# AIM-SE/AC-TSR

Measured on AMD Instinct MI355X. Metric: user-sequences/sec fwd+bwd, AC-SASRec L=50 d=64, 1/2/4/8 MI355X, higher is better.
Workload: dtype f32; 1 GPU; ACSASRec full training step (spatial + adversarial calibrators, BASELINE configs[2]), synthetic 100000-item catalogue, B=512/GPU L=50 d=64 h=2 2 layers inner=256, CE loss, two-pass backward + Adam; global_batch=512, seq_len=50, hidden=64, heads=2, parallelism=dp1, launch=hipGraph replay per step, backward=two walks (reference protocol, trainer.py:672-686)

## Files before the change

ac_tsr_amd/csrc/acattn_linear.hip:

```cpp
#include <stdlib.h>

#include <algorithm>

#include "acattn_common.h"
#include "acattn_sumrows.h"

namespace {

constexpr int kRegs = 64;

struct WgradGroup {
  const float* x[ACATTN_WGRAD_MAX_GROUP];
  const float* dy[ACATTN_WGRAD_MAX_GROUP];
  float* dw[ACATTN_WGRAD_MAX_GROUP];
  float* db[ACATTN_WGRAD_MAX_GROUP];
  int K[ACATTN_WGRAD_MAX_GROUP];
  int N[ACATTN_WGRAD_MAX_GROUP];
  long long w_off[ACATTN_WGRAD_MAX_GROUP];
  long long b_off[ACATTN_WGRAD_MAX_GROUP];
};

__device__ __forceinline__ f4 load_rows4(const float* base, int64_t row, int64_t M, int ld, int col, int ncols) {
  f4 v = {0.f, 0.f, 0.f, 0.f};
  if (row < M) {
    const float* p = base + row * ld + col;
    if (col + 3 < ncols) {
      v = *(const f4u*)p;
    } else {
#pragma unroll
      for (int e = 0; e < 4; ++e)
        if (col + e < ncols) v[e] = p[e];
    }
  }
  return v;
}

template <int UNROLL>
__global__ void __launch_bounds__(256, 2) wgrad_partial_kernel(const WgradGroup G, const int64_t M,
                                                             float* __restrict__ ws) {
  const int it = blockIdx.z;
  const int K = G.K[it], N = G.N[it];
  const int KB = (K + 63) >> 6, NB = (N + 63) >> 6;
  if ((int)blockIdx.y >= KB * NB) return;
  const float* __restrict__ x = G.x[it];
  const float* __restrict__ dy = G.dy[it];
  float* part_w = ws + G.w_off[it];
  float* part_b = G.db[it] ? ws + G.b_off[it] : nullptr;
  const int lane = threadIdx.x & 63, wave = threadIdx.x >> 6;
  const int c = lane & 15, g = lane >> 4;
  const int blk = blockIdx.y, nb = blk / KB, kb = blk - nb * KB;
  const int P = gridDim.x;
  const int ncol = nb * 64 + 4 * c, kcol = kb * 64 + 4 * c;

  f4 acc[4][4];
#pragma unroll
  for (int a = 0; a < 4; ++a)
#pragma unroll
    for (int b = 0; b < 4; ++b) acc[a][b] = f4{0.f, 0.f, 0.f, 0.f};
  f4 bsum = {0.f, 0.f, 0.f, 0.f};

  const int64_t stride = (int64_t)P * 4 * 4, batch = stride * UNROLL;
  int64_t m0 = ((int64_t)blockIdx.x * 4 + wave) * 4;
  if ((K & 63) == 0 && (N & 63) == 0) {
    auto load_batch = [&](int64_t r0, f4 (&xv)[UNROLL], f4 (&gv)[UNROLL]) {
#pragma unroll
      for (int u = 0; u < UNROLL; ++u) {
        const int64_t row = min(r0 + u * stride + g, M - 1);
        xv[u] = *(const f4*)(x + row * K + kcol);
        gv[u] = *(const f4*)(dy + row * N + ncol);
      }
    };
    auto mma_batch = [&](int64_t r0, const f4 (&xv)[UNROLL], const f4 (&gv)[UNROLL]) {
#pragma unroll
      for (int u = 0; u < UNROLL; ++u) {
        const bool row_in = r0 + u * stride + g < M;
        f4 gq;
#pragma unroll
        for (int e = 0; e < 4; ++e) gq[e] = row_in ? gv[u][e] : 0.f;
        bsum += gq;
#pragma unroll
        for (int a = 0; a < 4; ++a)
#pragma unroll
          for (int b = 0; b < 4; ++b) acc[a][b] = mfma16(gq[a], xv[u][b], acc[a][b]);
      }
    };
    f4 xa[UNROLL], ga[UNROLL], xb[UNROLL], gb[UNROLL];
    load_batch(m0, xa, ga);
#pragma nounroll
    for (; m0 < M; m0 += 2 * batch) {
      load_batch(m0 + batch, xb, gb);
      __builtin_amdgcn_sched_barrier(0);
      mma_batch(m0, xa, ga);
      load_batch(m0 + 2 * batch, xa, ga);
      __builtin_amdgcn_sched_barrier(0);
      if (m0 + batch < M) mma_batch(m0 + batch, xb, gb);
    }
  } else {
    for (; m0 < M; m0 += batch) {
      f4 xv[UNROLL], gv[UNROLL];
#pragma unroll
      for (int u = 0; u < UNROLL; ++u) {
        const int64_t row = m0 + u * stride + g;
        xv[u] = load_rows4(x, row, M, K, kcol, K);
        gv[u] = load_rows4(dy, row, M, N, ncol, N);
      }
#pragma unroll
      for (int u = 0; u < UNROLL; ++u) {
        bsum += gv[u];
#pragma unroll
        for (int a = 0; a < 4; ++a)
#pragma unroll
          for (int b = 0; b < 4; ++b) acc[a][b] = mfma16(gv[u][a], xv[u][b], acc[a][b]);
      }
    }
  }

  __shared__ float red[4 * kRegs * 64];
#pragma unroll
  for (int a = 0; a < 4; ++a)
#pragma unroll
    for (int b = 0; b < 4; ++b)
#pragma unroll
      for (int r = 0; r < 4; ++r) red[(wave * kRegs + (a * 4 + b) * 4 + r) * 64 + lane] = acc[a][b][r];
  __syncthreads();
  float* pw = part_w + ((size_t)blk * P + blockIdx.x) * (kRegs * 64);
  for (int s = threadIdx.x; s < kRegs * 64; s += 256)
    pw[s] = (red[s] + red[kRegs * 64 + s]) + (red[2 * kRegs * 64 + s] + red[3 * kRegs * 64 + s]);
  if (part_b && kb == 0) {
    __syncthreads();
    *(f4*)(red + 4 * threadIdx.x) = bsum;
    __syncthreads();
    if (threadIdx.x < 64) {
      float s = 0.f;
#pragma unroll
      for (int wg = 0; wg < 16; ++wg) s += red[4 * (wg * 16 + (threadIdx.x >> 2)) + (threadIdx.x & 3)];
      part_b[((size_t)nb * P + blockIdx.x) * 64 + threadIdx.x] = s;
    }
  }
}

__global__ void __launch_bounds__(256) wgrad_reduce_kernel(const WgradGroup G, const float* __restrict__ ws,
                                                            const int P) {
  const int it = blockIdx.z;
  const int K = G.K[it], N = G.N[it];
  const int KB = (K + 63) >> 6, NB = (N + 63) >> 6;
  if ((int)blockIdx.y >= KB * NB) return;
  float* __restrict__ dw = G.dw[it];
  float* __restrict__ db = G.db[it];
  const float* part_w = ws + G.w_off[it];
  const float* part_b = ws + G.b_off[it];
  const int blk = blockIdx.y, nb = blk / KB, kb = blk - nb * KB;
  const int sl = threadIdx.x & 31, q = threadIdx.x >> 5;
  const int s = blockIdx.x * 32 + sl;
  const float* pw = part_w + (size_t)blk * P * (kRegs * 64) + s;
  constexpr size_t PS = kRegs * 64;
  float a[8];
#pragma unroll
  for (int u = 0; u < 8; ++u) a[u] = 0.f;
  int p = q;
  for (; p + 56 < P; p += 64) {
#pragma unroll
    for (int u = 0; u < 8; ++u) a[u] += pw[(size_t)(p + 8 * u) * PS];
  }
  for (; p < P; p += 8) a[0] += pw[(size_t)p * PS];
  __shared__ float red[8][32];
  red[q][sl] = ((a[0] + a[1]) + (a[2] + a[3])) + ((a[4] + a[5]) + (a[6] + a[7]));
  __syncthreads();
  if (q == 0) {
    float v = 0.f;
#pragma unroll
    for (int u = 0; u < 8; ++u) v += red[u][sl];
    const int reg = s >> 6, lane = s & 63;
    const int tile = reg >> 2, r = reg & 3, aa = tile >> 2, bb = tile & 3, g = lane >> 4, c = lane & 15;
    const int n = nb * 64 + 4 * (4 * g + r) + aa, k = kb * 64 + 4 * c + bb;
    if (n < N && k < K) dw[(size_t)n * K + k] = v;
  }
  if (db && kb == 0 && blockIdx.x < 2) {
    __syncthreads();
    const int col = blockIdx.x * 32 + sl, nn = nb * 64 + col;
    const float* pb = part_b + (size_t)nb * P * 64 + col;
    float sb = 0.f;
    for (int t = q; t < P; t += 8) sb += pb[(size_t)t * 64];
    red[q][sl] = sb;
    __syncthreads();
    if (q == 0 && nn < N) {
      float v = 0.f;
#pragma unroll
      for (int u = 0; u < 8; ++u) v += red[u][sl];
      db[nn] = v;
    }
  }
}

struct WgradMany {
  const float* part_w[ACATTN_WGRAD_MAX_REDUCE];
  const float* part_b[ACATTN_WGRAD_MAX_REDUCE];
  float* dw[ACATTN_WGRAD_MAX_REDUCE];
  float* db[ACATTN_WGRAD_MAX_REDUCE];
  int K[ACATTN_WGRAD_MAX_REDUCE];
  int N[ACATTN_WGRAD_MAX_REDUCE];
  int P[ACATTN_WGRAD_MAX_REDUCE];
  SumRowsJob sr[ACATTN_SUMROWS_MAX_DEFER];
  int n_w;
};

__global__ void __launch_bounds__(256) wgrad_reduce_many_kernel(const WgradMany G) {
  if ((int)blockIdx.z >= G.n_w) {
    const SumRowsJob& j = G.sr[blockIdx.z - G.n_w];
    const int w = blockIdx.y * gridDim.x + blockIdx.x;
    if (w < j.n_wg) sum_rows_block<false>(j.x, j.out, j.R, j.C, j.R, j.CT, w % j.col_groups, 0, w / j.col_groups);
    return;
  }
  const int it = blockIdx.z;
  const int K = G.K[it], N = G.N[it];
  const int KB = (K + 63) >> 6, NB = (N + 63) >> 6;
  if ((int)blockIdx.y >= KB * NB) return;
  float* __restrict__ dw = G.dw[it];
  float* __restrict__ db = G.db[it];
  const float* part_w = G.part_w[it];
  const float* part_b = G.part_b[it];
  const int P = G.P[it];
  const int blk = blockIdx.y, nb = blk / KB, kb = blk - nb * KB;
  const int sl = threadIdx.x & 31, q = threadIdx.x >> 5;
  const int s = blockIdx.x * 32 + sl;
  const float* pw = part_w + (size_t)blk * P * (kRegs * 64) + s;
  constexpr size_t PS = kRegs * 64;
  float a[8];
#pragma unroll
  for (int u = 0; u < 8; ++u) a[u] = 0.f;
  int p = q;
  for (; p + 56 < P; p += 64) {
#pragma unroll
    for (int u = 0; u < 8; ++u) a[u] += pw[(size_t)(p + 8 * u) * PS];
  }
  for (; p < P; p += 8) a[0] += pw[(size_t)p * PS];
  __shared__ float red[8][32];
  red[q][sl] = ((a[0] + a[1]) + (a[2] + a[3])) + ((a[4] + a[5]) + (a[6] + a[7]));
  __syncthreads();
  if (q == 0) {
    float v = 0.f;
#pragma unroll
    for (int u = 0; u < 8; ++u) v += red[u][sl];
    const int reg = s >> 6, lane = s & 63;
    const int tile = reg >> 2, r = reg & 3, aa = tile >> 2, bb = tile & 3, g = lane >> 4, c = lane & 15;
    const int n = nb * 64 + 4 * (4 * g + r) + aa, k = kb * 64 + 4 * c + bb;
    if (n < N && k < K) dw[(size_t)n * K + k] = v;
  }
  if (db && kb == 0 && blockIdx.x < 2) {
    __syncthreads();
    const int col = blockIdx.x * 32 + sl, nn = nb * 64 + col;
    const float* pb = part_b + (size_t)nb * P * 64 + col;
    float sb = 0.f;
    for (int t = q; t < P; t += 8) sb += pb[(size_t)t * 64];
    red[q][sl] = sb;
    __syncthreads();
    if (q == 0 && nn < N) {
      float v = 0.f;
#pragma unroll
      for (int u = 0; u < 8; ++u) v += red[u][sl];
      db[nn] = v;
    }
  }
}

int pick_partials(int64_t M, int blocks) {
  static const int forced = getenv("ACATTN_WGRAD_PARTIALS") ? atoi(getenv("ACATTN_WGRAD_PARTIALS")) : 0;
  int p = forced > 0 ? forced : std::max(64, 128 / blocks);
  return (int)std::min<int64_t>(p, std::max<int64_t>(1, M / 64));
}

}

namespace {
int64_t item_ws_floats(int K, int N, int P) {
  const int64_t KB = (K + 63) / 64, NB = (N + 63) / 64;
  return KB * NB * P * kRegs * 64 + NB * P * 64;
}
int group_partials(int64_t M, const int* K, const int* N, int n_items) {
  int blocks = 1;
  for (int i = 0; i < n_items; ++i) blocks = std::max(blocks, ((K[i] + 63) / 64) * ((N[i] + 63) / 64));
  return pick_partials(M, blocks);
}
}

int64_t acattn_linear_wgrad_ws_bytes(int64_t M, int K, int N) {
  return item_ws_floats(K, N, pick_partials(M, 1)) * (int64_t)sizeof(float);
}

int acattn_launch_linear_wgrad(const float* const* x, const float* const* dy, const int* K, const int* N,
                               float* const* dw, float* const* db, int n_items, int64_t M, void* ws, hipStream_t stream,
                               int* P_out, long long* w_off_out, long long* b_off_out) {
  WgradGroup G{};
  const int P = group_partials(M, K, N, n_items);
  int blocks = 1;
  long long off = 0;
  for (int i = 0; i < n_items; ++i) {
    G.x[i] = x[i];
    G.dy[i] = dy[i];
    G.dw[i] = dw[i];
    G.db[i] = db[i];
    G.K[i] = K[i];
    G.N[i] = N[i];
    const long long KB = (K[i] + 63) / 64, NB = (N[i] + 63) / 64;
    G.w_off[i] = off;
    G.b_off[i] = off + KB * NB * P * kRegs * 64;
    off += item_ws_floats(K[i], N[i], P);
    blocks = std::max(blocks, (int)(KB * NB));
  }
  const int64_t groups_per_wave = ((M + 3) / 4 + (int64_t)P * 4 - 1) / ((int64_t)P * 4);
  const dim3 grid(P, blocks, n_items);
  if (groups_per_wave > 4)
    hipLaunchKernelGGL((wgrad_partial_kernel<5>), grid, dim3(256), 0, stream, G, M, (float*)ws);
  else if (groups_per_wave >= 4)
    hipLaunchKernelGGL((wgrad_partial_kernel<4>), grid, dim3(256), 0, stream, G, M, (float*)ws);
  else
    hipLaunchKernelGGL((wgrad_partial_kernel<1>), grid, dim3(256), 0, stream, G, M, (float*)ws);
  int rc = (int)hipGetLastError();
  if (rc) return rc;
  if (P_out) {
    *P_out = P;
    for (int i = 0; i < n_items; ++i) {
      w_off_out[i] = G.w_off[i];
      b_off_out[i] = G.b_off[i];
    }
    return 0;
  }
  hipLaunchKernelGGL(wgrad_reduce_kernel, dim3(kRegs * 2, blocks, n_items), dim3(256), 0, stream, G, (const float*)ws, P);
  return (int)hipGetLastError();
}

int acattn_launch_linear_wgrad_reduce_many(const float* const* part_w, const float* const* part_b, const int* K, const int* N,
                                           const int* P, float* const* dw, float* const* db, int n_items,
                                           const float* const* sr_x, float* const* sr_out, const int* sr_R, const int* sr_C,
                                           int n_sr, hipStream_t stream) {
  WgradMany G{};
  G.n_w = n_items;
  int blocks = 1;
  for (int i = 0; i < n_sr; ++i) {
    G.sr[i] = make_job(sr_x[i], sr_out[i], 1, sr_R[i], sr_C[i]);
    blocks = std::max(blocks, (G.sr[i].n_wg + kRegs * 2 - 1) / (kRegs * 2));
  }
  for (int i = 0; i < n_items; ++i) {
    G.part_w[i] = part_w[i];
    G.part_b[i] = part_b[i];
    G.dw[i] = dw[i];
    G.db[i] = db[i];
    G.K[i] = K[i];
    G.N[i] = N[i];
    G.P[i] = P[i];
    blocks = std::max(blocks, ((K[i] + 63) / 64) * ((N[i] + 63) / 64));
  }
  hipLaunchKernelGGL(wgrad_reduce_many_kernel, dim3(kRegs * 2, blocks, n_items + n_sr), dim3(256), 0, stream, G);
  return (int)hipGetLastError();
}
```

Baseline: 541,000 user-sequences/sec.

## Add split-precision MFMA weight-gradient kernel with double-buffered row slabs

Adds a weight-gradient partial kernel that splits f32 inputs into several low-precision parts and accumulates them with split MFMA products over 32-row slabs per wave. Slab loads are double-buffered behind scheduling barriers so memory fetches overlap the matrix math. It has its own partial-count heuristic. The kernel is chosen only when M is large enough, the total work is small enough, and the linear-products choice selects the split mode, so it may not run by default. The split emulation keeps f32 accuracy but adds extra conversion and MFMA work per element.

New measurement: 547,500 user-sequences/sec (median of 6 runs). +1.2%, better.

```diff
diff --git a/ac_tsr_amd/csrc/acattn_linear.hip b/ac_tsr_amd/csrc/acattn_linear.hip
--- a/ac_tsr_amd/csrc/acattn_linear.hip
+++ b/ac_tsr_amd/csrc/acattn_linear.hip
@@ -1,8 +1,10 @@
 #include <stdlib.h>
 
 #include <algorithm>
+#include <type_traits>
 
 #include "acattn_common.h"
+#include "acattn_split.h"
 #include "acattn_sumrows.h"
 
 namespace {
@@ -34,6 +36,9 @@
   }
   return v;
 }
+
+__device__ __forceinline__ void fold_and_store(const f4 (&acc)[4][4], const f4 bsum, float* part_w, float* part_b,
+                                               const int blk, const int nb, const int kb, const int P);
 
 template <int UNROLL>
 __global__ void __launch_bounds__(256, 2) wgrad_partial_kernel(const WgradGroup G, const int64_t M,
@@ -115,6 +120,107 @@
     }
   }
 
+  fold_and_store(acc, bsum, part_w, part_b, blk, nb, kb, P);
+}
+
+__global__ void __launch_bounds__(256, 1) wgrad_split_partial_kernel(const WgradGroup G, const int64_t M,
+                                                                   float* __restrict__ ws) {
+  const int it = blockIdx.z;
+  const int K = G.K[it], N = G.N[it];
+  const int KB = (K + 63) >> 6, NB = (N + 63) >> 6;
+  if ((int)blockIdx.y >= KB * NB) return;
+  const float* __restrict__ x = G.x[it];
+  const float* __restrict__ dy = G.dy[it];
+  float* part_w = ws + G.w_off[it];
+  float* part_b = G.db[it] ? ws + G.b_off[it] : nullptr;
+  const int lane = threadIdx.x & 63;
+  const int wave = __builtin_amdgcn_readfirstlane(threadIdx.x >> 6);
+  const int c = lane & 15, g = lane >> 4;
+  const int blk = blockIdx.y, nb = blk / KB, kb = blk - nb * KB;
+  const int P = gridDim.x;
+  const int ncol = nb * 64 + 4 * c, kcol = kb * 64 + 4 * c;
+
+  f4 acc[4][4];
+#pragma unroll
+  for (int a = 0; a < 4; ++a)
+#pragma unroll
+    for (int b = 0; b < 4; ++b) acc[a][b] = f4{0.f, 0.f, 0.f, 0.f};
+  f4 bsum = {0.f, 0.f, 0.f, 0.f};
+
+  const int xc = min(kcol, K - 4), gc = min(ncol, N - 4);
+  const int xsh = min(kcol - xc, 3), gsh = min(ncol - gc, 3);
+  auto load_slab = [&](int64_t r0, f4 (&xv)[8], f4 (&gv)[8]) {
+    if (r0 + 32 <= M) {
+      const float* px = x + (r0 + 8 * g) * K + xc;
+      const float* pg = dy + (r0 + 8 * g) * N + gc;
+#pragma unroll
+      for (int j = 0; j < 8; ++j) {
+        xv[j] = *(const f4u*)(px + j * K);
+        gv[j] = *(const f4u*)(pg + j * N);
+      }
+    } else if (r0 < M) {
+#pragma unroll
+      for (int j = 0; j < 8; ++j) {
+        const int64_t row = r0 + 8 * g + j, rr = min(row, M - 1);
+        xv[j] = *(const f4u*)(x + rr * K + xc);
+        const f4 t = *(const f4u*)(dy + rr * N + gc);
+        gv[j] = row < M ? t : f4{0.f, 0.f, 0.f, 0.f};
+      }
+    }
+  };
+  auto unshift = [&](const f4 v, const int sh) {
+    const f4 t = sh & 1 ? f4{v[1], v[2], v[3], v[3]} : v;
+    return sh & 2 ? f4{t[2], t[3], t[3], t[3]} : t;
+  };
+  auto mma_slab = [&](auto ragged, const f4 (&xv)[8], const f4 (&gv)[8]) {
+    b8 xp[4][3];
+#pragma unroll
+    for (int b = 0; b < 4; ++b) {
+      float t[8];
+#pragma unroll
+      for (int j = 0; j < 8; ++j) t[j] = ragged ? unshift(xv[j], xsh)[b] : xv[j][b];
+      split8(t, xp[b][0], xp[b][1], xp[b][2]);
+    }
+#pragma unroll
+    for (int a = 0; a < 4; ++a) {
+      float t[8];
+#pragma unroll
+      for (int j = 0; j < 8; ++j) {
+        t[j] = ragged ? unshift(gv[j], gsh)[a] : gv[j][a];
+        bsum[a] += t[j];
+      }
+      b8 gp[3];
+      split8(t, gp[0], gp[1], gp[2]);
+#pragma unroll
+      for (int b = 0; b < 4; ++b) acc[a][b] = mfma_split(gp, xp[b], acc[a][b]);
+    }
+  };
+
+  auto run = [&](auto ragged) {
+    const int64_t step = (int64_t)P * 4 * 32;
+    int64_t m0 = ((int64_t)blockIdx.x * 4 + wave) * 32;
+    f4 xa[8], ga[8], xb[8], gb[8];
+    load_slab(m0, xa, ga);
+#pragma nounroll
+    for (; m0 < M; m0 += 2 * step) {
+      load_slab(m0 + step, xb, gb);
+      __builtin_amdgcn_sched_barrier(0);
+      mma_slab(ragged, xa, ga);
+      load_slab(m0 + 2 * step, xa, ga);
+      __builtin_amdgcn_sched_barrier(0);
+      if (m0 + step < M) mma_slab(ragged, xb, gb);
+    }
+  };
+  if (((K | N) & 63) != 0)
+    run(std::true_type{});
+  else
+    run(std::false_type{});
+  fold_and_store(acc, bsum, part_w, part_b, blk, nb, kb, P);
+}
+
+__device__ __forceinline__ void fold_and_store(const f4 (&acc)[4][4], const f4 bsum, float* part_w, float* part_b,
+                                               const int blk, const int nb, const int kb, const int P) {
+  const int lane = threadIdx.x & 63, wave = threadIdx.x >> 6;
   __shared__ float red[4 * kRegs * 64];
 #pragma unroll
   for (int a = 0; a < 4; ++a)
@@ -269,6 +375,25 @@
   return (int)std::min<int64_t>(p, std::max<int64_t>(1, M / 64));
 }
 
+constexpr int kSIMDs = 1024, kSplitSlabsPerWave = 8, kSplitMinRows = 4096;
+bool use_split_wgrad(int64_t M, const int* K, const int* N, int n_items) {
+  int64_t work_blocks = 0;
+  for (int i = 0; i < n_items; ++i) {
+    if (K[i] < 4 || N[i] < 4) return false;
+    work_blocks += ((K[i] + 63) / 64) * ((N[i] + 63) / 64);
+  }
+  if (M < kSplitMinRows || work_blocks * ((M + 31) / 32) > (int64_t)kSplitSlabsPerWave * kSIMDs) return false;
+  return acattn_linear_products_choice(-1) == 1;
+}
+
+int pick_split_partials(int64_t M, int blocks, int work_blocks) {
+  static const int forced = getenv("ACATTN_WGRAD_PARTIALS") ? atoi(getenv("ACATTN_WGRAD_PARTIALS")) : 0;
+  const int upper = pick_partials(M, blocks);
+  if (forced > 0) return upper;
+  const int p = std::max(16, 256 / std::max(1, work_blocks));
+  return (int)std::min<int64_t>(std::min(p, upper), std::max<int64_t>(1, M / 128));
+}
+
 }
 
 namespace {
@@ -276,10 +401,14 @@
   const int64_t KB = (K + 63) / 64, NB = (N + 63) / 64;
   return KB * NB * P * kRegs * 64 + NB * P * 64;
 }
-int group_partials(int64_t M, const int* K, const int* N, int n_items) {
-  int blocks = 1;
-  for (int i = 0; i < n_items; ++i) blocks = std::max(blocks, ((K[i] + 63) / 64) * ((N[i] + 63) / 64));
-  return pick_partials(M, blocks);
+int group_partials(int64_t M, const int* K, const int* N, int n_items, bool split) {
+  int blocks = 1, work_blocks = 0;
+  for (int i = 0; i < n_items; ++i) {
+    const int b = ((K[i] + 63) / 64) * ((N[i] + 63) / 64);
+    blocks = std::max(blocks, b);
+    work_blocks += b;
+  }
+  return split ? pick_split_partials(M, blocks, work_blocks) : pick_partials(M, blocks);
 }
 }
 
@@ -291,7 +420,8 @@
                                float* const* dw, float* const* db, int n_items, int64_t M, void* ws, hipStream_t stream,
                                int* P_out, long long* w_off_out, long long* b_off_out) {
   WgradGroup G{};
-  const int P = group_partials(M, K, N, n_items);
+  const bool split = use_split_wgrad(M, K, N, n_items);
+  const int P = group_partials(M, K, N, n_items, split);
   int blocks = 1;
   long long off = 0;
   for (int i = 0; i < n_items; ++i) {
@@ -309,7 +439,9 @@
   }
   const int64_t groups_per_wave = ((M + 3) / 4 + (int64_t)P * 4 - 1) / ((int64_t)P * 4);
   const dim3 grid(P, blocks, n_items);
-  if (groups_per_wave > 4)
+  if (split)
+    hipLaunchKernelGGL(wgrad_split_partial_kernel, grid, dim3(256), 0, stream, G, M, (float*)ws);
+  else if (groups_per_wave > 4)
     hipLaunchKernelGGL((wgrad_partial_kernel<5>), grid, dim3(256), 0, stream, G, M, (float*)ws);
   else if (groups_per_wave >= 4)
     hipLaunchKernelGGL((wgrad_partial_kernel<4>), grid, dim3(256), 0, stream, G, M, (float*)ws);
```
